# mhozza/covest

Measured on AMD Instinct MI355X. Metric: grid-point log-likelihood evals/s, repeat model, 10k-bin hist, higher is better.
Workload: dtype f64

## Files before the change

### covest_amd/_capi.py

```python
import ctypes
import os
import sys

_HERE = os.path.dirname(os.path.abspath(__file__))
LIB_PATH = os.environ.get("COVEST_AMD_LIB", os.path.join(_HERE, "lib", "libcovest_amd.so"))

MAX_PARAMS = 5
MODEL_BASIC, MODEL_REPEATS = 0, 1
KERNEL_AUTO, KERNEL_DIRECT, KERNEL_RECUR, KERNEL_FACTORED, KERNEL_DIRECT_REF = 0, 1, 2, 3, 4
KERNELS = {"auto": KERNEL_AUTO, "direct": KERNEL_DIRECT, "recur": KERNEL_RECUR,
           "factored": KERNEL_FACTORED, "direct_ref": KERNEL_DIRECT_REF}

EXPORTS = (
    "covest_abi_version", "covest_device_count", "covest_last_error",
    "covest_model_create", "covest_model_destroy", "covest_model_param_count",
    "covest_model_bins_evaluated", "covest_threshold_o", "covest_eval_points", "covest_eval_points_grad", "covest_eval_points_hess",
    "covest_eval_points_opg",
    "covest_probabilities", "covest_reference_overflow", "covest_grid_create", "covest_grid_reset", "covest_grid_destroy", "covest_grid_size",
    "covest_grid_eval", "covest_grid_eval_scan", "covest_grid_scan", "covest_grid_argmin", "covest_grid_axis_min", "covest_grid_argmin_pair_device",
    "covest_grid_ll_device",
    "covest_grid_ll_host",
    "covest_grid_work", "covest_grid_profile", "covest_grid_kernel_ms", "covest_grid_diag",
    "covest_grid_launch_record", "covest_model_launch_record", "covest_compiled_variants",
    "covest_kmer_create", "covest_kmer_destroy", "covest_kmer_reserve", "covest_kmer_add",
    "covest_kmer_add_device", "covest_kmer_histogram", "covest_kmer_slots", "covest_kmer_clear",
    "covest_kmer_count_reads_device", "covest_kmer_partition_info", "covest_kmer_partition_ms", "covest_kmer_memory_limit",
    "covest_kmer_scatter_rate",
    "covest_reads_open", "covest_reads_close", "covest_reads_next", "covest_reads_bytes",
    "covest_thin_histogram", "covest_thin_histogram_timed",
    "covest_truncated_poisson", "covest_truncated_poisson_table",
    "covest_random_genome", "covest_random_genome_device", "covest_simulate_reads", "covest_simulate_reads_device",
    "covest_sample_reads", "covest_sample_reads_device",
    "covest_repeat_plan", "covest_repeat_genome", "covest_repeat_genome_device",
    "covest_draw_thresholds", "covest_draw_histograms", "covest_draw_histograms_device",
    "covest_batch_create", "covest_batch_draw", "covest_batch_counts", "covest_batch_eval_cross", "covest_batch_eval_pairs",
    "covest_batch_argmin_cross", "covest_batch_info", "covest_batch_destroy",
# ... 100 lines not shown
    L.covest_grid_eval.argtypes = [vp, i32, vp]
    L.covest_grid_eval_scan.restype = ctypes.c_int
    L.covest_grid_eval_scan.argtypes = [vp, i32, vp, ctypes.c_double]
    L.covest_grid_scan.restype = ctypes.c_int
    L.covest_grid_scan.argtypes = [vp, i32, ctypes.POINTER(i64), dp, ctypes.POINTER(i32), ctypes.POINTER(i32)]
    L.covest_grid_argmin.restype = ctypes.c_int
    L.covest_grid_argmin.argtypes = [vp, dp, ctypes.POINTER(i64)]
    L.covest_grid_axis_min.restype = ctypes.c_int
    L.covest_grid_axis_min.argtypes = [vp, ctypes.c_uint32, i64, dp, ctypes.POINTER(i64)]
    L.covest_grid_argmin_pair_device.restype = vp
    L.covest_grid_argmin_pair_device.argtypes = [vp]
    L.covest_grid_ll_device.restype = vp
    L.covest_grid_ll_device.argtypes = [vp]
    L.covest_grid_ll_host.restype = ctypes.c_int
    L.covest_grid_ll_host.argtypes = [vp, dp]
    L.covest_grid_work.restype = ctypes.c_int
    L.covest_grid_work.argtypes = [vp, dp, dp, ctypes.POINTER(ctypes.c_char_p)]
    L.covest_grid_profile.restype = ctypes.c_int
    L.covest_grid_profile.argtypes = [vp, i32]
    L.covest_grid_kernel_ms.restype = ctypes.c_int
    L.covest_grid_kernel_ms.argtypes = [vp, dp, ctypes.POINTER(i64)]
    u8p = ctypes.POINTER(ctypes.c_uint8)
    i64p = ctypes.POINTER(i64)
    L.covest_kmer_create.restype = ctypes.c_int
    L.covest_kmer_create.argtypes = [i32, i32, i64, i32, ctypes.POINTER(vp)]
    L.covest_kmer_destroy.restype = None
    L.covest_kmer_destroy.argtypes = [vp]
    L.covest_kmer_reserve.restype = ctypes.c_int
    L.covest_kmer_reserve.argtypes = [vp, i64]
    L.covest_kmer_add.restype = ctypes.c_int
# ... 167 lines not shown
```

### covest_amd/csrc/abi_grid.cpp

```cpp
#include "host.h"

using namespace covest;

namespace covest {

int grid_stage_begin(covest_grid *g, size_t bytes, StageSlot &slot)
{
    if (!g->async_uploads) {
        SharedStage &ss = shared_stage();
        slot.shared_hold = std::unique_lock<std::mutex>(ss.mu);
        HIP_TRY(ss.buf.reserve(bytes));
        slot.ptr = ss.buf.as<char>();
        return COVEST_OK;
    }
    const size_t at = (g->stage_off + 63) / 64 * 64;
    if (at + bytes > g->stage.cap) {
        if (g->stage.ptr)
            g->stage_retired.push_back(std::move(g->stage));
        HIP_TRY(g->stage.reserve(std::max<size_t>(2 * (at + bytes), 1 << 18)));
        slot.ptr = g->stage.as<char>();
        g->stage_off = bytes;
        return COVEST_OK;
    }
    slot.ptr = g->stage.as<char>() + at;
// ... 139 lines not shown

}

static int grid_configure(covest_grid *g, int32_t n_axes, const double *const *axes, const int64_t *axis_len,
                          int64_t flat_begin, int64_t flat_end, const char *who)
{
    covest_model *m = g->model;
    int64_t total = 0, n_values = 0;
    const int arc = check_grid_args(m, n_axes, axes, axis_len, flat_begin, &flat_end, who, &total, &n_values);
    if (arc != COVEST_OK)
        return arc;
    g->configured = false;
    g->flat_begin = flat_begin;
    g->flat_end = flat_end;
    g->evaluated = false;
    g->scan_valid = false;
    g->ev_used = 0;
    g->stage_off = 0;
    const int64_t n = flat_end - flat_begin;
    const int64_t n1 = n_axes == 5 ? axis_len[2] : 1, n2 = n_axes == 5 ? axis_len[3] : 1, n3 = n_axes == 5 ? axis_len[4] : 1;
    const int64_t nq = n_axes == 5 ? n1 * n2 * n3 : 0;

    std::vector<int32_t> table((size_t)nq);
    if (nq)
        threshold_table(m, axes[2], n1, axes[3], n2, axes[4], n3, table.data());

    const GridArena arena(n_values, nq, n);
    char *inputs = nullptr;
    const int src = stage_inputs(g, arena, n_axes, axes, axis_len, table, n, &inputs);
    if (src != COVEST_OK)
// ... 194 lines not shown
    double tsum = 0;
    long long hist[6] = {0, 0, 0, 0, 0, 0};
    for (int64_t i : idx) {
        const long long T = tt[(size_t)((g->src.flat_begin + i) % n_q)];
        tmin = std::min(tmin, T);
        tmax = std::max(tmax, T);
        tsum += (double)T;
        hist[T <= 16 ? 0 : T <= 32 ? 1 : T <= 64 ? 2 : T <= 128 ? 3 : T <= 256 ? 4 : 5]++;
    }
    std::fprintf(stderr, "covest_grid_eval: threshold_o of the queued points: min %lld mean %.1f max %lld; <=16 %lld <=32 %lld <=64 %lld <=128 %lld <=256 %lld more %lld\n",
                 tmin, tsum / queued, tmax, hist[0], hist[1], hist[2], hist[3], hist[4], hist[5]);
    return COVEST_OK;
}
#endif

static int grid_eval(covest_grid *g, int32_t kernel, void *stream, bool scan, double scan_start)
{
    if (!g)
        return fail(COVEST_E_INVALID, "covest_grid_eval: null grid");
    if (!g->configured)
        return fail(COVEST_E_INVALID, "covest_grid_eval: the last covest_grid_reset of this handle failed; reset it again");
    covest_model *m = g->model;
    const int kern = resolve_kernel(m, kernel, g);
    if (kern < 0)
        return kern;
    std::lock_guard<std::mutex> guard(m->lock);
    DeviceGuard dev_guard(m->device);
    int rc = dev_guard.status();
    if (rc != COVEST_OK)
        return rc;
    LaunchRecordScope record(g->record);
    hipStream_t st = static_cast<hipStream_t>(stream);
    const int64_t n = g->flat_end - g->flat_begin;
    if (g->upload_pending && st != nullptr && g->upload_ev)
        HIP_TRY(hipStreamWaitEvent(st, g->upload_ev, 0));
    hipEvent_t bracket_end = nullptr;
    rc = bracket_begin(g, st, &bracket_end);
    if (rc != COVEST_OK)
        return rc;
    HIP_TRY(launch_ll(m, kern, g->src, n, g->ll.as<double>(), sub_list_of(m, g->has_plan ? g->t_max : 2, g->sub_index.ptr, g->sub_word.ptr, g->sub_ctl.ptr), st,
                      &g->last_kernel, g));
    g->last_kernel_id = kern;
    if (bracket_end)
        HIP_TRY(hipEventRecord(bracket_end, st));
#ifdef COVEST_DIAG
    rc = report_queue(g, st, n);
    if (rc != COVEST_OK)
        return rc;
#endif
    if (!g->result_host) {
        static_assert(sizeof(ArgminResult) <= 64 && 64 + sizeof(ScanRecords) <= kPinnedBlockBytes, "pinned block");
        g->result_host = static_cast<ArgminResult *>(pinned_block_take());
        if (!g->result_host)
            return fail(COVEST_E_NOMEM, "covest_grid_eval: no page-locked memory for the result");
    }
    g->scan_valid = scan && n >= 1 && n <= kArgminSmall;
    if (g->scan_valid)
        HIP_TRY(launch_argmin_scan(g->ll.as<double>(), n, g->flat_begin, scan_start, g->result.as<ArgminResult>(), g->result_host,
                                   g->scan_host(), g->sub_ctl.as<unsigned>(), st));
    else
        HIP_TRY(launch_argmin(g->ll.as<double>(), n, g->flat_begin, g->partial_val.as<double>(),
                              g->partial_idx.as<int64_t>(), g->result.as<ArgminResult>(), g->result_host, g->sub_ctl.as<unsigned>(), st));
    g->last_stream = st;
    g->evaluated = true;
    return COVEST_OK;
}

int covest_grid_eval(covest_grid *g, int32_t kernel, void *stream) { return grid_eval(g, kernel, stream, false, 0.0); }

int covest_grid_eval_scan(covest_grid *g, int32_t kernel, void *stream, double start_min)
{
    return grid_eval(g, kernel, stream, true, start_min);
}

int covest_grid_scan(covest_grid *g, int32_t cap, int64_t *index, double *negll, int32_t *n_records, int32_t *truncated)
{
    if (!g || !n_records || !truncated || cap < 0 || (cap > 0 && (!index || !negll)))
        return fail(COVEST_E_INVALID, "covest_grid_scan: bad argument");
    if (!g->evaluated)
        return fail(COVEST_E_INVALID, "covest_grid_scan: covest_grid_eval_scan has not run");
    DeviceGuard dev_guard(g->model->device);
    int rc = dev_guard.status();
    if (rc != COVEST_OK)
        return rc;
    HIP_TRY(hipStreamSynchronize(g->last_stream));
    *n_records = 0;
    *truncated = 1;
// ... 3 lines not shown
    const int32_t have = sr->n;
    *truncated = (sr->truncated || have > cap) ? 1 : 0;
    const int32_t take = std::min(have, cap);
    for (int32_t i = 0; i < take; ++i) {
        index[i] = sr->rec[i].index;
        negll[i] = sr->rec[i].negll;
    }
    *n_records = take;
    return COVEST_OK;
}

int64_t covest_grid_launch_record(const covest_grid *g, char *buf, int64_t cap)
{
    if (!g || cap < 0 || (cap > 0 && !buf))
        return fail(COVEST_E_INVALID, "covest_grid_launch_record: bad argument");
    return launch_record_text(g->record, buf, cap);
}

int covest_grid_argmin(covest_grid *g, double *min_negll, int64_t *argmin_flat)
{
    if (!g || !min_negll || !argmin_flat)
        return fail(COVEST_E_INVALID, "covest_grid_argmin: null argument");
    if (!g->evaluated)
        return fail(COVEST_E_INVALID, "covest_grid_argmin: covest_grid_eval has not run");
    DeviceGuard dev_guard(g->model->device);
    int rc = dev_guard.status();
    if (rc != COVEST_OK)
        return rc;
    HIP_TRY(hipStreamSynchronize(g->last_stream));
    const ArgminResult r = *g->result_host;
    *min_negll = r.min_negll;
    *argmin_flat = r.index < 0 ? -1 : g->flat_begin + r.index;
    return COVEST_OK;
}

int covest_grid_axis_min(covest_grid *g, uint32_t keep_mask, int64_t n_cells, double *min_negll, int64_t *argmin_flat)
{
    if (!g || !min_negll || !argmin_flat)
        return fail(COVEST_E_INVALID, "covest_grid_axis_min: null argument");
    if (!g->evaluated)
        return fail(COVEST_E_INVALID, "covest_grid_axis_min: covest_grid_eval has not run");
    covest_model *m = g->model;
    if (keep_mask >> m->n_par)
        return fail(COVEST_E_INVALID, "covest_grid_axis_min: keep_mask names an axis the grid does not have");
// ... 6 lines not shown
    std::lock_guard<std::mutex> guard(m->lock);
    DeviceGuard dev_guard(m->device);
    int rc = dev_guard.status();
    if (rc != COVEST_OK)
        return rc;
    AxisMinPlan p;
    if (!axis_min_plan(g->len, m->n_par, keep_mask, g->flat_begin, g->flat_end, &p))
        return fail(COVEST_E_INVALID, "covest_grid_axis_min: the axes do not fit a plan");
    const size_t nc = (size_t)n_cells, n_part = p.n_slices > 1 ? nc * (size_t)p.n_slices : 0;
    HIP_TRY(g->axis_buf.reserve(16 * (nc + n_part)));
    double *out_v = g->axis_buf.as<double>();
    int64_t *out_i = reinterpret_cast<int64_t *>(out_v + nc);
    double *part_v = reinterpret_cast<double *>(out_i + nc);
    int64_t *part_i = reinterpret_cast<int64_t *>(part_v + n_part);
    hipStream_t st = g->last_stream;
    HIP_TRY(launch_axis_min(p, g->ll.as<double>(), part_v, part_i, out_v, out_i, st));
    if (16 * nc <= ((size_t)1 << 20)) {
        HIP_TRY(g->axis_host.reserve(16 * nc));
        HIP_TRY(hipMemcpyAsync(g->axis_host.ptr, out_v, 16 * nc, hipMemcpyDeviceToHost, st));
        HIP_TRY(hipStreamSynchronize(st));
        std::memcpy(min_negll, g->axis_host.ptr, 8 * nc);
        std::memcpy(argmin_flat, static_cast<char *>(g->axis_host.ptr) + 8 * nc, 8 * nc);
    } else {
        HIP_TRY(hipStreamSynchronize(st));
        HIP_TRY(hipMemcpy(min_negll, out_v, 8 * nc, hipMemcpyDeviceToHost));
        HIP_TRY(hipMemcpy(argmin_flat, out_i, 8 * nc, hipMemcpyDeviceToHost));
    }
    return COVEST_OK;
}

const double *covest_grid_ll_device(const covest_grid *g) { return g ? g->ll.as<double>() : nullptr; }

const double *covest_grid_argmin_pair_device(const covest_grid *g)
{
    return g ? g->result.as<ArgminResult>()->pair : nullptr;
}

int covest_grid_ll_host(covest_grid *g, double *out_ll)
{
    if (!g || !out_ll)
        return fail(COVEST_E_INVALID, "covest_grid_ll_host: null argument");
    if (!g->evaluated)
        return fail(COVEST_E_INVALID, "covest_grid_ll_host: covest_grid_eval has not run");
    DeviceGuard dev_guard(g->model->device);
    int rc = dev_guard.status();
    if (rc != COVEST_OK)
        return rc;
    const int64_t n = g->flat_end - g->flat_begin;
    HIP_TRY(hipStreamSynchronize(g->last_stream));
    if (n > 0)
        HIP_TRY(hipMemcpy(out_ll, g->ll.ptr, (size_t)n * sizeof(double), hipMemcpyDeviceToHost));
    return COVEST_OK;
}

int64_t covest_grid_diag(covest_grid *g, int64_t *out, int64_t n)
{
    if (!g || !g->has_plan || !g->plan.diag)
        return 0;
// ... 39 lines not shown
```

### covest_amd/csrc/abi_model.cpp

```cpp
#include "host.h"

using namespace covest;

static int check_model_desc(const covest_model_desc *d)
{
    if (d->kind != COVEST_MODEL_BASIC && d->kind != COVEST_MODEL_REPEATS)
        return fail(COVEST_E_INVALID, "covest_model_create: unknown model kind");
    if (d->n_err < 1 || d->n_err > COVEST_MAX_ERROR_CLASSES || d->n_err > d->k + 1)
        return fail(COVEST_E_INVALID, "covest_model_create: n_err must be in 1..min(k+1, 64)");
    if (d->r <= 0 || d->k <= 0)
        return fail(COVEST_E_INVALID, "covest_model_create: k and r must be positive");
    if (d->n_keys < 0 || (d->n_keys > 0 && (!d->keys || !d->counts)) || !d->comb)
        return fail(COVEST_E_INVALID, "covest_model_create: null histogram or comb");
    if (d->kind == COVEST_MODEL_REPEATS && d->n_keys == 0)
        return fail(COVEST_E_INVALID,
                    "covest_model_create: repeats model needs a non-empty histogram "
                    "(max() of an empty dict raises in covest/models.py:186)");
    return COVEST_OK;
}

static void fill_dev_model(DevModel &dm, const covest_model_desc *d, int n_par)
{
    dm.kind = d->kind;
    dm.k = d->k;
// ... 159 lines not shown
        return COVEST_KERNEL_DIRECT_REF;
    case COVEST_KERNEL_RECUR:
        if (basic_fast)
            return COVEST_KERNEL_RECUR;
        return fail(COVEST_E_INVALID, "recurrence kernel needs the basic model, max_error <= 32 and keys in 1..16384");
    case COVEST_KERNEL_FACTORED:
        if (factored_ok || (!g && m->has_tiles && m->dm.kind == COVEST_MODEL_REPEATS && m->dm.n_err <= 8))
            return COVEST_KERNEL_FACTORED;
        return fail(COVEST_E_INVALID, "factored kernel needs the repeats model, keys in 1..16384 and max_error <= 32 "
                                      "(<= 8 for a point list)");
    default:
        return fail(COVEST_E_INVALID, "unknown kernel");
    }
}

static hipError_t launch_factored_grid(covest_grid *g, double *out, const SubList &sub, hipStream_t st)
{
    const covest_model *m = g->model;
    if (g->has_short_part) {
        record_factored_plan(g->plan, g->n_shared_tiles, false);
        hipError_t e = launch_ll_factored(m->dm, m->tv, g->plan, out, sub, st);
        if (e != hipSuccess)
            return e;
        e = launch_ll_fix_list(m->dm, m->tv, g->src, out, sub, st, g->flat_end - g->flat_begin);
        if (e != hipSuccess)
            return e;
    }
    if (g->n_long_tiles > 0) {
        const int64_t n_cols = (int64_t)g->n_long_tiles * 16, n_rows = (int64_t)m->tv.n_items * kTileBins;
        const int64_t ce_begin = g->plan.ce_begin, ce_end = g->plan.ce_end;
        const int64_t per_ce = n_cols * n_rows * (int64_t)sizeof(double);
        const int64_t batch = std::max<int64_t>(1, std::min<int64_t>(ce_end - ce_begin, ((int64_t)1 << 30) / per_ce));
        hipError_t e = g->long_partial.reserve((size_t)(batch * per_ce));
        if (e != hipSuccess)
            return e;
        for (const covest_grid::Part &part : g->long_parts)
            record_factored_plan(part.plan, 0, true);
        for (int64_t first = ce_begin; first < ce_end; first += batch) {
            const int64_t last = std::min(ce_end, first + batch);
// ... 21 lines not shown
{
    SubList l{};
    l.p_clamp = clamp_for(m, t_max);
    l.log_p_clamp = std::log(l.p_clamp);
    l.count = static_cast<unsigned *>(ctl);
    l.index = static_cast<int64_t *>(index);
    l.word = static_cast<unsigned long long *>(word);
    l.index_offset = 0;
#ifdef COVEST_DIAG
    const char *dc = std::getenv("COVEST_DIAG_BASIC_CLASS");
    l.diag_class = dc ? std::atoi(dc) : 0;
#endif
    return l;
}

hipError_t launch_ll(const covest_model *m, int kernel, const PointSource &src, int64_t n, double *out, const SubList &sub,
                     hipStream_t st, const char **name, const covest_grid *g)
{
    if (kernel == COVEST_KERNEL_FACTORED) {
        if (name)
            *name = "ll_factored";
        return launch_factored_grid(const_cast<covest_grid *>(g), out, sub, st);
    }
    if (kernel == COVEST_KERNEL_RECUR) {
        if (name)
            *name = "ll_basic";
        hipError_t e = launch_ll_basic(m->dm, m->tv, src, n, out, sub, st);
        return e != hipSuccess ? e : launch_ll_fix_list(m->dm, m->tv, src, out, sub, st, n);
    }
    if (name)
        *name = kernel == COVEST_KERNEL_DIRECT_REF ? "ll_direct_ref" : "ll_direct";
    return launch_ll_direct(m->dm, src, n, out, nullptr, st, kernel == COVEST_KERNEL_DIRECT_REF);
}

}

constexpr int64_t kInPlaceMaxListPoints = 4;

static int reserve_point_queue(covest_model *m, int64_t n)
{
    HIP_TRY(m->ws_sub_index.reserve((size_t)n * sizeof(int64_t)));
    HIP_TRY(m->ws_sub_word.reserve((size_t)n * sizeof(unsigned long long)));
    HIP_TRY(m->ws_sub_ctl.reserve(sizeof(unsigned)));
    HIP_TRY(hipMemsetAsync(m->ws_sub_ctl.ptr, 0, sizeof(unsigned), nullptr));
    return COVEST_OK;
}

// ... 406 lines not shown
```

### covest_amd/csrc/argmin.hip

```cpp
#include <hip/hip_runtime.h>

#include <algorithm>

#include "cand.h"
#include "kernels.h"
#include "wave.h"

namespace covest {

namespace {

__device__ __forceinline__ Cand block_best(Cand c)
{
    __shared__ double sv[16];
    __shared__ int64_t si[16];
    c = wave_best(c);
    const int lane = threadIdx.x & (kWave - 1), w = threadIdx.x / kWave;
    if (lane == 0) {
        sv[w] = c.v;
        si[w] = c.i;
    }
    __syncthreads();
    const int n_w = blockDim.x / kWave;
    Cand r;
// ... 12 lines not shown
    for (int64_t i = (int64_t)blockIdx.x * blockDim.x + threadIdx.x; i < n; i += stride) {
        const double v = -ll[i];
        if (v < c.v) {
            c.v = v;
            c.i = i;
        }
    }
    c = block_best(c);
    if (threadIdx.x == 0) {
        pv[blockIdx.x] = c.v;
        pi[blockIdx.x] = c.i;
    }
}

__device__ __forceinline__ void publish(Cand c, int64_t flat_begin, ArgminResult *__restrict__ result,
                                        ArgminResult *__restrict__ host_mirror)
{
    ArgminResult r;
    r.min_negll = c.v;
    r.index = (c.i == INT64_MAX) ? -1 : c.i;
    r.pair[0] = c.v;
    r.pair[1] = (c.i == INT64_MAX) ? -1.0 : (double)(flat_begin + c.i);
    *result = r;
    if (host_mirror)
        *host_mirror = r;
}

__global__ __launch_bounds__(256) void argmin_stage2(const double *__restrict__ pv,
                                                     const int64_t *__restrict__ pi, int n_part, int64_t flat_begin,
                                                     ArgminResult *__restrict__ result, ArgminResult *__restrict__ host_mirror,
                                                     unsigned *__restrict__ queue_count)
{
    if (threadIdx.x == 0 && queue_count)
        *queue_count = 0;
    Cand c;
    c.v = INFINITY;
    c.i = INT64_MAX;
    for (int i = threadIdx.x; i < n_part; i += blockDim.x) {
        Cand o;
        o.v = pv[i];
        o.i = pi[i];
        c = better(c, o);
    }
    c = block_best(c);
    if (threadIdx.x == 0)
        publish(c, flat_begin, result, host_mirror);
}

constexpr int kSmallThreads = 1024;

template <class Take>
__device__ __forceinline__ void small_grid_values(const double *__restrict__ ll, int64_t n, Take take)
{
    for (int64_t base = threadIdx.x; base < n; base += 4 * kSmallThreads) {
        double v[4];
#pragma unroll
        for (int u = 0; u < 4; ++u) {
            const int64_t i = base + (int64_t)u * kSmallThreads;
            v[u] = i < n ? -ll[i] : INFINITY;
        }
#pragma unroll
        for (int u = 0; u < 4; ++u) {
            const int64_t i = base + (int64_t)u * kSmallThreads;
            if (i < n)
                take(i, v[u]);
        }
    }
}

__global__ __launch_bounds__(kSmallThreads) void argmin_small(const double *__restrict__ ll, int64_t n, int64_t flat_begin,
                                                             ArgminResult *__restrict__ result, ArgminResult *__restrict__ host_mirror,
                                                             unsigned *__restrict__ queue_count)
{
    if (threadIdx.x == 0 && queue_count)
        *queue_count = 0;
    Cand c;
    c.v = INFINITY;
    c.i = INT64_MAX;
    small_grid_values(ll, n, [&](int64_t i, double v) {
        if (v < c.v) {
            c.v = v;
            c.i = i;
        }
    });
    c = block_best(c);
    if (threadIdx.x == 0)
        publish(c, flat_begin, result, host_mirror);
}

__global__ __launch_bounds__(kSmallThreads) void argmin_scan_small(const double *__restrict__ ll, int64_t n, int64_t flat_begin,
                                                                  double start, ArgminResult *__restrict__ result,
                                                                  ArgminResult *__restrict__ host_mirror,
                                                                  ScanRecords *__restrict__ scan, unsigned *__restrict__ queue_count)
{
    constexpr int NW = kSmallThreads / kWave;
    extern __shared__ double vals[];
    __shared__ double wave_min[NW];
    __shared__ int wave_cnt[NW];
    const int tid = threadIdx.x, lane = tid & (kWave - 1), w = tid / kWave;
    if (tid == 0 && queue_count)
        *queue_count = 0;
    Cand c;
// ... 91 lines not shown
                                           hipFuncAttributeMaxDynamicSharedMemorySize, (int)(kArgminSmall * sizeof(double)));
        if (e != hipSuccess)
            return e;
        raised[dev] = true;
    }
    record_launch(kArgminVariantNames[2]);
    hipLaunchKernelGGL(argmin_scan_small, dim3(1), dim3(kSmallThreads), lds, stream, ll, n, flat_begin, start, result, host_mirror, scan,
                       queue_count);
    return hipGetLastError();
}


hipError_t launch_argmin(const double *ll, int64_t n, int64_t flat_begin, double *partial_val, int64_t *partial_idx,
                         ArgminResult *result, ArgminResult *host_mirror, unsigned *queue_count, hipStream_t stream)
{
    if (n <= kArgminSmall) {
        record_launch(kArgminVariantNames[0]);
        hipLaunchKernelGGL(argmin_small, dim3(1), dim3(kSmallThreads), 0, stream, ll, n, flat_begin, result, host_mirror, queue_count);
        return hipGetLastError();
    }
    const int blocks = (int)std::min<int64_t>(kArgminBlocks, std::max<int64_t>(1, (n + 255) / 256));
    record_launch(kArgminVariantNames[1]);
    hipLaunchKernelGGL(argmin_stage1, dim3(blocks), dim3(256), 0, stream, ll, n, partial_val, partial_idx);
    hipLaunchKernelGGL(argmin_stage2, dim3(1), dim3(256), 0, stream, partial_val, partial_idx, blocks, flat_begin, result,
                       host_mirror, queue_count);
    return hipGetLastError();
}

}
```

### covest_amd/csrc/host.h

```cpp
#pragma once
#include <hip/hip_runtime.h>

#include <algorithm>
#include <cmath>
#include <cstdio>
#include <cstdlib>
#include <cstring>
#include <deque>
#include <limits>
#include <mutex>
#include <new>
#include <optional>
#include <string>
#include <vector>

#include "../../include/covest_amd.h"
#include "device_model.h"
#include "handback.h"
#include "kernels.h"

namespace covest {

int set_error(int code, const std::string &msg);
inline int fail(int code, const std::string &msg) { return set_error(code, msg); }
// ... 227 lines not shown
    int32_t n_shared_tiles = 0;
    std::vector<int32_t> long_q_orig_host;
    DevBuf long_q_orig, long_partial;
    int t_max = 2;
    double q_sum_t_minus_1 = 0.0;
    double contract_flops_per_row = 0.0;
    double sum_t_minus_1 = 0.0;
    LaunchRecord record;
    const char *last_kernel = "none";
    int last_kernel_id = 0;
    hipStream_t last_stream = nullptr;
    ArgminResult *result_host = nullptr;
    ScanRecords *scan_host() const { return reinterpret_cast<ScanRecords *>(reinterpret_cast<char *>(result_host) + 64); }
    bool scan_valid = false;
    bool counter_clean = false;
    HostBuf stage;
    std::vector<HostBuf> stage_retired;
    size_t stage_off = 0;
    bool async_uploads = false;
    bool upload_pending = false;
    hipEvent_t upload_ev = nullptr;
    bool evaluated = false;
    bool configured = false;
    bool profiling = false;
    std::vector<hipEvent_t> ev_begin, ev_end;
    size_t ev_used = 0;
};


struct BulkState {
// ... 62 lines not shown
static_assert(kListLanes + 1 == 513, "include/covest_amd.h documents the largest threshold_o of an uncut point");
double copy_number_weight_host(double q1, double q2, double q, int o);
int build_factored_plan(covest_grid *g, const double *const *axes, const int64_t *axis_len,
                        const std::vector<int32_t> &t_table);
int build_list_plan(covest_model *m, int64_t n, const double *params, const std::vector<int32_t> &t_list,
                    const std::vector<int32_t> *o_base_list, DevBuf &buf, FactoredPlan &pl, bool in_place = false);

int draw_histograms_resident(const char *who, int64_t m, const double *weights, int64_t n_draws, int64_t first_rep,
                             int64_t n_rep, uint64_t seed, DevBuf &d_thr, DevBuf &d_out);

constexpr int64_t kInPlaceMaxPoints = 256;
int resolve_kernel(const covest_model *m, int32_t kernel, const covest_grid *g);
SubList sub_list_of(const covest_model *m, int t_max, void *index, void *word, void *ctl);
hipError_t launch_ll(const covest_model *m, int kernel, const PointSource &src, int64_t n, double *out, const SubList &sub,
                     hipStream_t st, const char **name, const covest_grid *g = nullptr);

}
```

### covest_amd/csrc/host_common.cpp

```cpp
#include "host.h"

using namespace covest;

namespace {
thread_local std::string g_last_error;
}

namespace covest {

int set_error(int code, const std::string &msg)
{
    g_last_error = msg;
    return code;
}

int fail_hip(hipError_t e, const char *what)
{
    g_last_error = std::string(what) + ": " + hipGetErrorString(e);
    if (e == hipErrorOutOfMemory) {
        (void)hipGetLastError();
        return COVEST_E_NOMEM;
    }
    return (e == hipErrorNoDevice || e == hipErrorInvalidDevice || e == hipErrorInsufficientDriver)
               ? COVEST_E_NO_DEVICE
// ... 253 lines not shown
double lgamma_of_factorial(int64_t j)
{
    lgamma_ensure(j);
    return lgamma_at(j);
}

namespace {
thread_local LaunchRecord *tls_record = nullptr;
}

LaunchRecordScope::LaunchRecordScope(LaunchRecord &r) : prev(tls_record)
{
    r.clear();
    tls_record = &r;
}
LaunchRecordScope::~LaunchRecordScope() { tls_record = prev; }

void record_launch(const char *name, int64_t launches)
{
    LaunchRecord *r = tls_record;
    if (!r || launches <= 0)
        return;
    for (int i = 0; i < r->n_entries; ++i)
        if (r->entries[i].name == name) {
            r->entries[i].launches += launches;
            return;
        }
    if (r->n_entries < (int)(sizeof r->entries / sizeof r->entries[0]))
        r->entries[r->n_entries++] = LaunchRecord::Entry{name, launches};
}
// ... 88 lines not shown
```

### covest_amd/csrc/kernels.h

```cpp
#pragma once
#include <hip/hip_runtime_api.h>

#include <cstddef>

#include "device_model.h"
#include "handback.h"
#include "kmer_plan.h"
#include "tiles.h"

namespace covest {

struct LaunchRecord {
    struct Entry {
        const char *name;
        int64_t launches;
    };
    struct Plan {
        int32_t n_threads, n_buf, ld, n_qblocks, shared_tiles, n_pass, list_mode;
        bool long_part;
    };
    Entry entries[16];
    int n_entries = 0;
    Plan plans[8];
    int n_plans = 0;
    void clear() { n_entries = n_plans = 0; }
};
void record_launch(const char *name, int64_t launches = 1);
void record_factored_plan(const FactoredPlan &plan, int shared_tiles, bool long_part);
struct LaunchRecordScope {
    explicit LaunchRecordScope(LaunchRecord &r);
    ~LaunchRecordScope();
    LaunchRecord *prev;
};
constexpr int kFactoredVariants = 10, kBasicVariants = 8, kFixVariants = 6, kArgminVariants = 3, kDerivVariants = 7;
extern const char *const kFactoredVariantNames[kFactoredVariants];
extern const char *const kFactoredFinishNames[2];
extern const char *const kBasicVariantNames[kBasicVariants];
extern const char *const kFixVariantNames[kFixVariants];
extern const char *const kArgminVariantNames[kArgminVariants];
extern const char *const kDerivVariantNames[kDerivVariants];

hipError_t launch_ll_direct(const DevModel &m, const PointSource &src, int64_t n, double *out_ll,
                            double *out_p, hipStream_t stream, bool ref_overflow = false);

hipError_t launch_ll_basic(const DevModel &m, const TileView &tv, const PointSource &src, int64_t n,
// ... 6 lines not shown
                                     const int32_t *first_item, const double *point_par, const int32_t *point_T,
                                     int64_t n_points, double *out_ll, hipStream_t stream);

hipError_t launch_ll_finish_dense(const DevModel &m, const TileView &tv, const PointSource &src, const double *partial,
                                  int64_t ce_first, int64_t n_ce, int64_t n_cols, const int32_t *q_orig, int64_t n_q,
                                  int64_t flat_end, double *out_ll, hipStream_t stream);

hipError_t launch_ll_fix_list(const DevModel &m, const TileView &tv, const PointSource &src, double *ll,
                              const SubList &list, hipStream_t stream, int64_t n_points = 0);

constexpr int kArgminBlocks = 1024;
struct ArgminResult {
    double min_negll;
    int64_t index;
    double pair[2];
};
constexpr int64_t kArgminSmall = 16384;
hipError_t launch_argmin(const double *ll, int64_t n, int64_t flat_begin, double *partial_val, int64_t *partial_idx,
                         ArgminResult *result, ArgminResult *host_mirror, unsigned *queue_count, hipStream_t stream);

constexpr int kScanCap = 120;
struct ScanRecords {
    int32_t n;
    int32_t truncated;
    double start;
    struct {
        int64_t index;
        double negll;
    } rec[kScanCap];
};
hipError_t launch_argmin_scan(const double *ll, int64_t n, int64_t flat_begin, double start, ArgminResult *result,
                              ArgminResult *host_mirror, ScanRecords *scan, unsigned *queue_count, hipStream_t stream);

struct AxisMinPlan {
// ... 171 lines not shown
```

### covest_amd/grid.py

```python
import ctypes
import itertools
import math
import random

import numpy as np

from . import _capi, constants

_DP = ctypes.POINTER(ctypes.c_double)


def partition_flat_range(total, world_size, weights=None, period=None):
    if world_size < 1:
        raise ValueError("world_size must be >= 1")
    if weights is None or total == 0:
        return [(total * r) // world_size for r in range(world_size + 1)]
    w = np.asarray(weights, dtype=np.float64)
    period = len(w) if period is None else period
    assert period == len(w) and total % period == 0
    prefix = np.concatenate(([0.0], np.cumsum(w)))
    per_period = prefix[-1]
    n_periods = total // period
    whole = per_period * n_periods
    bounds = [0]
# ... 97 lines not shown
    return best, arg


class DenseGrid:

    def __init__(self, model, axes, flat_range=None):
        if len(axes) != model.param_count:
            raise ValueError("need one axis per model parameter")
        self.model = model
        ptrs, lens = self._take_axes(axes, flat_range)
        L = _capi.lib()
        h = ctypes.c_void_p()
        _capi.check(L.covest_grid_create(model.handle, len(self.axes), ptrs.ctypes.data, lens.ctypes.data, self.flat_range[0],
                                         self.flat_range[1], ctypes.byref(h)), "covest_grid_create")
        self._handle = h
        if hasattr(model, "_register_grid"):
            model._register_grid(self)

    def _take_axes(self, axes, flat_range):
        parts = [a if type(a) is np.ndarray and a.dtype == np.float64 and a.ndim == 1
                 else np.asarray(a, dtype=np.float64).reshape(-1) for a in axes]
        lens = [p.shape[0] for p in parts]
        flat = np.concatenate(parts) if len(parts) > 1 else np.ascontiguousarray(parts[0])
        self._flat = flat
        self.axes, offs, at = [], [], 0
        for n in lens:
            self.axes.append(flat[at:at + n])
            offs.append(at)
            at += n
        self.shape = tuple(lens)
# ... 58 lines not shown

    def axis_minima(self, keep):
        mask, picked = resolve_keep(self.model.params, keep)
        shape = tuple(self.shape[i] for i in picked)
        val = np.empty(shape, dtype=np.float64)
        idx = np.empty(shape, dtype=np.int64)
        _capi.check(_capi.lib().covest_grid_axis_min(self._handle, mask, val.size, val.ctypes.data_as(_DP),
                                                     idx.ctypes.data_as(ctypes.POINTER(ctypes.c_int64))),
                    "covest_grid_axis_min")
        return val, idx

    def loglikelihoods(self):
        out = np.empty(len(self), dtype=np.float64)
        _capi.check(_capi.lib().covest_grid_ll_host(self._handle, out.ctypes.data_as(_DP)),
                    "covest_grid_ll_host")
        return out

    @property
    def ll_device_ptr(self):
        return _capi.lib().covest_grid_ll_device(self._handle)

    def argmin_pair_tensor(self, device_index):
        import torch
        _capi.require_shared_runtime("DenseGrid.argmin_pair_tensor")
        ptr = _capi.lib().covest_grid_argmin_pair_device(self._handle)

        class _View:
            __cuda_array_interface__ = {"shape": (2,), "typestr": "<f8", "data": (int(ptr), False), "version": 2}

        return torch.as_tensor(_View(), device=torch.device("cuda", device_index))
# ... 247 lines not shown
```

### include/covest_amd.h

```cpp
#ifndef COVEST_AMD_H
#define COVEST_AMD_H

#include <stdint.h>

#ifdef __cplusplus
extern "C" {
#endif

#define COVEST_ABI_VERSION 1

#define COVEST_MODEL_BASIC 0
#define COVEST_MODEL_REPEATS 1
#define COVEST_MAX_PARAMS 5
#define COVEST_MAX_ERROR_CLASSES 64

#define COVEST_OK 0
#define COVEST_E_INVALID (-1)
#define COVEST_E_NO_DEVICE (-2)
#define COVEST_E_HIP (-3)
#define COVEST_E_NOMEM (-4)
#define COVEST_E_UNSUPPORTED (-5)

#define COVEST_KERNEL_AUTO 0
#define COVEST_KERNEL_DIRECT 1
// ... 52 lines not shown
int covest_truncated_poisson(int32_t device, int64_t n, const double *l, const int64_t *j, int32_t mode, double *out);
int covest_truncated_poisson_table(int32_t device, int64_t n_l, const double *l, int64_t n_j, const int64_t *j, double *out);

int covest_probabilities(covest_model *m, const double *params, int32_t clamp, double *out_p);

int covest_grid_create(covest_model *m, int32_t n_axes, const double *const *axes,
                       const int64_t *axis_len, int64_t flat_begin, int64_t flat_end,
                       covest_grid **out);
void covest_grid_destroy(covest_grid *g);
int covest_grid_reset(covest_grid *g, int32_t n_axes, const double *const *axes, const int64_t *axis_len,
                      int64_t flat_begin, int64_t flat_end);
int64_t covest_grid_size(const covest_grid *g);

int covest_grid_eval(covest_grid *g, int32_t kernel, void *stream);

int covest_grid_argmin(covest_grid *g, double *min_negll, int64_t *argmin_flat);

int covest_grid_axis_min(covest_grid *g, uint32_t keep_mask, int64_t n_cells, double *min_negll, int64_t *argmin_flat);

int covest_grid_eval_scan(covest_grid *g, int32_t kernel, void *stream, double start_min);
int covest_grid_scan(covest_grid *g, int32_t cap, int64_t *index, double *negll, int32_t *n_records, int32_t *truncated);

const double *covest_grid_argmin_pair_device(const covest_grid *g);

const double *covest_grid_ll_device(const covest_grid *g);
int covest_grid_ll_host(covest_grid *g, double *out_ll);

int covest_grid_work(const covest_grid *g, double *pmf_terms, double *flops, const char **kernel);

int64_t covest_grid_launch_record(const covest_grid *g, char *buf, int64_t cap);
// ... 90 lines not shown
```

Baseline: 396.1 million.

## Defer the strict fix-list pass until a consumer needs exact log-likelihoods

For recurrence and factored-with-short-part kernels, the grid eval now skips the fix-list relaunch over queued (numerically unsafe) points. Instead, the argmin kernel checks whether any queued point could threaten the provisional winner and flags the result as unproven. The fix pass plus a re-run of argmin then happens lazily, only when the argmin is unproven or the caller reads the log-likelihood arrays, axis mins or the device pair. This adds API surface, a 1024-thread stage2 that scans the queue, and lazy-completion bookkeeping that every accessor must honour.

Result: faster. 413.3 million (median of 6 runs) (+4.4%).

```diff
diff --git a/covest_amd/_capi.py b/covest_amd/_capi.py
--- a/covest_amd/_capi.py
+++ b/covest_amd/_capi.py
@@ -19,7 +19,7 @@
     "covest_probabilities", "covest_reference_overflow", "covest_grid_create", "covest_grid_reset", "covest_grid_destroy", "covest_grid_size",
     "covest_grid_eval", "covest_grid_eval_scan", "covest_grid_scan", "covest_grid_argmin", "covest_grid_axis_min", "covest_grid_argmin_pair_device",
     "covest_grid_ll_device",
-    "covest_grid_ll_host",
+    "covest_grid_ll_host", "covest_grid_complete", "covest_grid_fix_eager", "covest_grid_ll_provisional_host",
     "covest_grid_work", "covest_grid_profile", "covest_grid_kernel_ms", "covest_grid_diag",
     "covest_grid_launch_record", "covest_model_launch_record", "covest_compiled_variants",
     "covest_kmer_create", "covest_kmer_destroy", "covest_kmer_reserve", "covest_kmer_add",
@@ -150,6 +150,12 @@
     L.covest_grid_ll_device.argtypes = [vp]
     L.covest_grid_ll_host.restype = ctypes.c_int
     L.covest_grid_ll_host.argtypes = [vp, dp]
+    L.covest_grid_complete.restype = ctypes.c_int
+    L.covest_grid_complete.argtypes = [vp]
+    L.covest_grid_fix_eager.restype = ctypes.c_int
+    L.covest_grid_fix_eager.argtypes = [vp, ctypes.c_int32]
+    L.covest_grid_ll_provisional_host.restype = ctypes.c_int
+    L.covest_grid_ll_provisional_host.argtypes = [vp, dp]
     L.covest_grid_work.restype = ctypes.c_int
     L.covest_grid_work.argtypes = [vp, dp, dp, ctypes.POINTER(ctypes.c_char_p)]
     L.covest_grid_profile.restype = ctypes.c_int
diff --git a/covest_amd/csrc/abi_grid.cpp b/covest_amd/csrc/abi_grid.cpp
--- a/covest_amd/csrc/abi_grid.cpp
+++ b/covest_amd/csrc/abi_grid.cpp
@@ -177,6 +177,7 @@
     g->flat_begin = flat_begin;
     g->flat_end = flat_end;
     g->evaluated = false;
+    g->fix_pending = false;
     g->scan_valid = false;
     g->ev_used = 0;
     g->stage_off = 0;
@@ -401,6 +402,45 @@
 }
 #endif
 
+static SubList grid_queue(const covest_grid *g, bool put_off)
+{
+    return sub_list_of(g->model, g->has_plan ? g->t_max : 2, g->sub_index.ptr, g->sub_word.ptr,
+                       g->sub_ctl.as<unsigned>() + (put_off ? 1 : 0));
+}
+
+static int grid_complete(covest_grid *g, bool *launched = nullptr)
+{
+    if (launched)
+        *launched = false;
+    if (!g->fix_pending)
+        return COVEST_OK;
+    const covest_model *m = g->model;
+    const int64_t n = g->flat_end - g->flat_begin;
+    hipStream_t st = g->last_stream;
+    LaunchRecordScope record(g->record, true);
+    HIP_TRY(launch_ll_fix_list(m->dm, m->tv, g->src, g->ll.as<double>(), grid_queue(g, true), st, n));
+    HIP_TRY(launch_argmin(g->ll.as<double>(), n, g->flat_begin, g->partial_val.as<double>(), g->partial_idx.as<int64_t>(),
+                          g->result.as<ArgminResult>(), g->result_host, nullptr, st));
+    g->fix_pending = false;
+    if (launched)
+        *launched = true;
+    return COVEST_OK;
+}
+
+static int grid_complete_entry(covest_grid *g, bool *launched = nullptr)
+{
+    if (launched)
+        *launched = false;
+    if (!g->fix_pending)
+        return COVEST_OK;
+    covest_model *m = g->model;
+    std::lock_guard<std::mutex> guard(m->lock);
+    DeviceGuard dev_guard(m->device);
+    if (dev_guard.status() != COVEST_OK)
+        return dev_guard.status();
+    return grid_complete(g, launched);
+}
+
 static int grid_eval(covest_grid *g, int32_t kernel, void *stream, bool scan, double scan_start)
 {
     if (!g)
@@ -421,12 +461,16 @@
     const int64_t n = g->flat_end - g->flat_begin;
     if (g->upload_pending && st != nullptr && g->upload_ev)
         HIP_TRY(hipStreamWaitEvent(st, g->upload_ev, 0));
+    g->fix_pending = false;
+    g->counter_clean = false;
+    const bool hands_back = kern == COVEST_KERNEL_RECUR || (kern == COVEST_KERNEL_FACTORED && g->has_short_part);
+    const bool put_off = hands_back && !scan && !g->fix_eager;
     hipEvent_t bracket_end = nullptr;
     rc = bracket_begin(g, st, &bracket_end);
     if (rc != COVEST_OK)
         return rc;
-    HIP_TRY(launch_ll(m, kern, g->src, n, g->ll.as<double>(), sub_list_of(m, g->has_plan ? g->t_max : 2, g->sub_index.ptr, g->sub_word.ptr, g->sub_ctl.ptr), st,
-                      &g->last_kernel, g));
+    HIP_TRY((put_off ? launch_ll_unfixed : launch_ll)(m, kern, g->src, n, g->ll.as<double>(), grid_queue(g, false), st,
+                                                      &g->last_kernel, g));
     g->last_kernel_id = kern;
     if (bracket_end)
         HIP_TRY(hipEventRecord(bracket_end, st));
@@ -446,8 +490,11 @@
         HIP_TRY(launch_argmin_scan(g->ll.as<double>(), n, g->flat_begin, scan_start, g->result.as<ArgminResult>(), g->result_host,
                                    g->scan_host(), g->sub_ctl.as<unsigned>(), st));
     else
-        HIP_TRY(launch_argmin(g->ll.as<double>(), n, g->flat_begin, g->partial_val.as<double>(),
-                              g->partial_idx.as<int64_t>(), g->result.as<ArgminResult>(), g->result_host, g->sub_ctl.as<unsigned>(), st));
+        HIP_TRY(launch_argmin_proving(g->ll.as<double>(), n, g->flat_begin, g->partial_val.as<double>(),
+                                      g->partial_idx.as<int64_t>(), g->result.as<ArgminResult>(), g->result_host,
+                                      g->sub_ctl.as<unsigned>(), put_off ? g->sub_index.as<int64_t>() : nullptr, st));
+    g->counter_clean = true;
+    g->fix_pending = put_off;
     g->last_stream = st;
     g->evaluated = true;
     return COVEST_OK;
@@ -458,6 +505,22 @@
 int covest_grid_eval_scan(covest_grid *g, int32_t kernel, void *stream, double start_min)
 {
     return grid_eval(g, kernel, stream, true, start_min);
+}
+
+int covest_grid_complete(covest_grid *g)
+{
+    if (!g)
+        return fail(COVEST_E_INVALID, "covest_grid_complete: null grid");
+    return grid_complete_entry(g);
+}
+
+int covest_grid_fix_eager(covest_grid *g, int32_t eager)
+{
+    if (!g)
+        return fail(COVEST_E_INVALID, "covest_grid_fix_eager: null grid");
+    COVEST_TRY(grid_complete_entry(g));
+    g->fix_eager = eager != 0;
+    return COVEST_OK;
 }
 
 int covest_grid_scan(covest_grid *g, int32_t cap, int64_t *index, double *negll, int32_t *n_records, int32_t *truncated)
@@ -491,6 +554,7 @@
 {
     if (!g || cap < 0 || (cap > 0 && !buf))
         return fail(COVEST_E_INVALID, "covest_grid_launch_record: bad argument");
+    COVEST_TRY(grid_complete_entry(const_cast<covest_grid *>(g)));
     return launch_record_text(g->record, buf, cap);
 }
 
@@ -505,6 +569,10 @@
     if (rc != COVEST_OK)
         return rc;
     HIP_TRY(hipStreamSynchronize(g->last_stream));
+    if (g->fix_pending && g->result_host->unproven != 0) {
+        COVEST_TRY(grid_complete_entry(g));
+        HIP_TRY(hipStreamSynchronize(g->last_stream));
+    }
     const ArgminResult r = *g->result_host;
     *min_negll = r.min_negll;
     *argmin_flat = r.index < 0 ? -1 : g->flat_begin + r.index;
@@ -541,6 +609,7 @@
     double *part_v = reinterpret_cast<double *>(out_i + nc);
     int64_t *part_i = reinterpret_cast<int64_t *>(part_v + n_part);
     hipStream_t st = g->last_stream;
+    COVEST_TRY(grid_complete(g));
     HIP_TRY(launch_axis_min(p, g->ll.as<double>(), part_v, part_i, out_v, out_i, st));
     if (16 * nc <= ((size_t)1 << 20)) {
         HIP_TRY(g->axis_host.reserve(16 * nc));
@@ -556,11 +625,30 @@
     return COVEST_OK;
 }
 
-const double *covest_grid_ll_device(const covest_grid *g) { return g ? g->ll.as<double>() : nullptr; }
+const double *covest_grid_ll_device(const covest_grid *g)
+{
+    if (!g)
+        return nullptr;
+    bool launched = false;
+    if (grid_complete_entry(const_cast<covest_grid *>(g), &launched) != COVEST_OK)
+        return nullptr;
+    if (launched) {
+        DeviceGuard dev_guard(g->model->device);
+        if (dev_guard.status() != COVEST_OK || hipStreamSynchronize(g->last_stream) != hipSuccess)
+            return nullptr;
+    }
+    return g->ll.as<double>();
+}
 
 const double *covest_grid_argmin_pair_device(const covest_grid *g)
 {
-    return g ? g->result.as<ArgminResult>()->pair : nullptr;
+    if (!g)
+        return nullptr;
+    covest_grid *gm = const_cast<covest_grid *>(g);
+    if (grid_complete_entry(gm) != COVEST_OK)
+        return nullptr;
+    gm->fix_eager = true;
+    return g->result.as<ArgminResult>()->pair;
 }
 
 int covest_grid_ll_host(covest_grid *g, double *out_ll)
@@ -569,6 +657,24 @@
         return fail(COVEST_E_INVALID, "covest_grid_ll_host: null argument");
     if (!g->evaluated)
         return fail(COVEST_E_INVALID, "covest_grid_ll_host: covest_grid_eval has not run");
+    DeviceGuard dev_guard(g->model->device);
+    int rc = dev_guard.status();
+    if (rc != COVEST_OK)
+        return rc;
+    const int64_t n = g->flat_end - g->flat_begin;
+    COVEST_TRY(grid_complete_entry(g));
+    HIP_TRY(hipStreamSynchronize(g->last_stream));
+    if (n > 0)
+        HIP_TRY(hipMemcpy(out_ll, g->ll.ptr, (size_t)n * sizeof(double), hipMemcpyDeviceToHost));
+    return COVEST_OK;
+}
+
+int covest_grid_ll_provisional_host(covest_grid *g, double *out_ll)
+{
+    if (!g || !out_ll)
+        return fail(COVEST_E_INVALID, "covest_grid_ll_provisional_host: null argument");
+    if (!g->evaluated || !g->fix_pending)
+        return fail(COVEST_E_INVALID, "covest_grid_ll_provisional_host: no strict pass is owed for the last evaluation");
     DeviceGuard dev_guard(g->model->device);
     int rc = dev_guard.status();
     if (rc != COVEST_OK)
diff --git a/covest_amd/csrc/abi_model.cpp b/covest_amd/csrc/abi_model.cpp
--- a/covest_amd/csrc/abi_model.cpp
+++ b/covest_amd/csrc/abi_model.cpp
@@ -197,7 +197,7 @@
     }
 }
 
-static hipError_t launch_factored_grid(covest_grid *g, double *out, const SubList &sub, hipStream_t st)
+static hipError_t launch_factored_grid(covest_grid *g, double *out, const SubList &sub, hipStream_t st, bool with_fix)
 {
     const covest_model *m = g->model;
     if (g->has_short_part) {
@@ -205,7 +205,8 @@
         hipError_t e = launch_ll_factored(m->dm, m->tv, g->plan, out, sub, st);
         if (e != hipSuccess)
             return e;
-        e = launch_ll_fix_list(m->dm, m->tv, g->src, out, sub, st, g->flat_end - g->flat_begin);
+        if (with_fix)
+            e = launch_ll_fix_list(m->dm, m->tv, g->src, out, sub, st, g->flat_end - g->flat_begin);
         if (e != hipSuccess)
             return e;
     }
@@ -257,23 +258,35 @@
     return l;
 }
 
-hipError_t launch_ll(const covest_model *m, int kernel, const PointSource &src, int64_t n, double *out, const SubList &sub,
-                     hipStream_t st, const char **name, const covest_grid *g)
+static hipError_t launch_ll_with(const covest_model *m, int kernel, const PointSource &src, int64_t n, double *out,
+                                 const SubList &sub, hipStream_t st, const char **name, const covest_grid *g, bool with_fix)
 {
     if (kernel == COVEST_KERNEL_FACTORED) {
         if (name)
             *name = "ll_factored";
-        return launch_factored_grid(const_cast<covest_grid *>(g), out, sub, st);
+        return launch_factored_grid(const_cast<covest_grid *>(g), out, sub, st, with_fix);
     }
     if (kernel == COVEST_KERNEL_RECUR) {
         if (name)
             *name = "ll_basic";
         hipError_t e = launch_ll_basic(m->dm, m->tv, src, n, out, sub, st);
-        return e != hipSuccess ? e : launch_ll_fix_list(m->dm, m->tv, src, out, sub, st, n);
+        return e != hipSuccess || !with_fix ? e : launch_ll_fix_list(m->dm, m->tv, src, out, sub, st, n);
     }
     if (name)
         *name = kernel == COVEST_KERNEL_DIRECT_REF ? "ll_direct_ref" : "ll_direct";
     return launch_ll_direct(m->dm, src, n, out, nullptr, st, kernel == COVEST_KERNEL_DIRECT_REF);
+}
+
+hipError_t launch_ll(const covest_model *m, int kernel, const PointSource &src, int64_t n, double *out, const SubList &sub,
+                     hipStream_t st, const char **name, const covest_grid *g)
+{
+    return launch_ll_with(m, kernel, src, n, out, sub, st, name, g, true);
+}
+
+hipError_t launch_ll_unfixed(const covest_model *m, int kernel, const PointSource &src, int64_t n, double *out,
+                             const SubList &sub, hipStream_t st, const char **name, const covest_grid *g)
+{
+    return launch_ll_with(m, kernel, src, n, out, sub, st, name, g, false);
 }
 
 }
diff --git a/covest_amd/csrc/argmin.hip b/covest_amd/csrc/argmin.hip
--- a/covest_amd/csrc/argmin.hip
+++ b/covest_amd/csrc/argmin.hip
@@ -50,11 +50,12 @@
 }
 
 __device__ __forceinline__ void publish(Cand c, int64_t flat_begin, ArgminResult *__restrict__ result,
-                                        ArgminResult *__restrict__ host_mirror)
+                                        ArgminResult *__restrict__ host_mirror, bool unproven = false)
 {
     ArgminResult r;
     r.min_negll = c.v;
     r.index = (c.i == INT64_MAX) ? -1 : c.i;
+    r.unproven = unproven ? 1 : 0;
     r.pair[0] = c.v;
     r.pair[1] = (c.i == INT64_MAX) ? -1.0 : (double)(flat_begin + c.i);
     *result = r;
@@ -62,13 +63,62 @@
         *host_mirror = r;
 }
 
-__global__ __launch_bounds__(256) void argmin_stage2(const double *__restrict__ pv,
+__device__ __forceinline__ void take_queue(unsigned *__restrict__ queue_count, unsigned *s_queued)
+{
+    if (threadIdx.x != 0)
+        return;
+    unsigned q = 0;
+    if (queue_count) {
+        q = queue_count[0];
+        queue_count[1] = q;
+        queue_count[0] = 0;
+    }
+    *s_queued = q;
+}
+
+__device__ __forceinline__ bool winner_unproven(Cand c, const double *__restrict__ ll, const int64_t *__restrict__ queue_index,
+                                                const unsigned *s_queued)
+{
+    __shared__ double win_v;
+    __shared__ int64_t win_i;
+    if (threadIdx.x == 0) {
+        win_v = c.v;
+        win_i = c.i;
+    }
+    __syncthreads();
+    const double v_w = win_v;
+    const int64_t i_w = win_i;
+    const unsigned queued = *s_queued;
+    int threat = 0;
+    if (i_w != INT64_MAX) {
+        const double bound = v_w + 1e-9 * fabs(v_w);
+        for (unsigned base = threadIdx.x; base < queued; base += 4 * blockDim.x) {
+            int64_t i[4];
+            double v[4];
+#pragma unroll
+            for (int u = 0; u < 4; ++u) {
+                const unsigned q = base + (unsigned)u * blockDim.x;
+                i[u] = q < queued ? queue_index[q] : -1;
+            }
+#pragma unroll
+            for (int u = 0; u < 4; ++u)
+                v[u] = i[u] >= 0 ? -ll[i[u]] : INFINITY;
+#pragma unroll
+            for (int u = 0; u < 4; ++u)
+                threat |= (v[u] <= bound || i[u] == i_w) ? 1 : 0;
+        }
+    }
+    return __syncthreads_or(threat) != 0;
+}
+
+__global__ __launch_bounds__(1024) void argmin_stage2(const double *__restrict__ ll, const int64_t *__restrict__ queue_index,
+                                                     const double *__restrict__ pv,
                                                      const int64_t *__restrict__ pi, int n_part, int64_t flat_begin,
                                                      ArgminResult *__restrict__ result, ArgminResult *__restrict__ host_mirror,
                                                      unsigned *__restrict__ queue_count)
 {
-    if (threadIdx.x == 0 && queue_count)
-        *queue_count = 0;
+    __shared__ unsigned s_queued;
+    take_queue(queue_count, &s_queued);
     Cand c;
     c.v = INFINITY;
     c.i = INT64_MAX;
@@ -79,8 +129,9 @@
         c = better(c, o);
     }
     c = block_best(c);
+    const bool unproven = queue_index ? winner_unproven(c, ll, queue_index, &s_queued) : false;
     if (threadIdx.x == 0)
-        publish(c, flat_begin, result, host_mirror);
+        publish(c, flat_begin, result, host_mirror, unproven);
 }
 
 constexpr int kSmallThreads = 1024;
@@ -106,10 +157,10 @@
 
 __global__ __launch_bounds__(kSmallThreads) void argmin_small(const double *__restrict__ ll, int64_t n, int64_t flat_begin,
                                                              ArgminResult *__restrict__ result, ArgminResult *__restrict__ host_mirror,
-                                                             unsigned *__restrict__ queue_count)
-{
-    if (threadIdx.x == 0 && queue_count)
-        *queue_count = 0;
+                                                             unsigned *__restrict__ queue_count, const int64_t *__restrict__ queue_index)
+{
+    __shared__ unsigned s_queued;
+    take_queue(queue_count, &s_queued);
     Cand c;
     c.v = INFINITY;
     c.i = INT64_MAX;
@@ -120,8 +171,9 @@
         }
     });
     c = block_best(c);
+    const bool unproven = queue_index ? winner_unproven(c, ll, queue_index, &s_queued) : false;
     if (threadIdx.x == 0)
-        publish(c, flat_begin, result, host_mirror);
+        publish(c, flat_begin, result, host_mirror, unproven);
 }
 
 __global__ __launch_bounds__(kSmallThreads) void argmin_scan_small(const double *__restrict__ ll, int64_t n, int64_t flat_begin,
@@ -243,16 +295,26 @@
 hipError_t launch_argmin(const double *ll, int64_t n, int64_t flat_begin, double *partial_val, int64_t *partial_idx,
                          ArgminResult *result, ArgminResult *host_mirror, unsigned *queue_count, hipStream_t stream)
 {
+    return launch_argmin_proving(ll, n, flat_begin, partial_val, partial_idx, result, host_mirror, queue_count, nullptr, stream);
+}
+
+hipError_t launch_argmin_proving(const double *ll, int64_t n, int64_t flat_begin, double *partial_val, int64_t *partial_idx,
+                                 ArgminResult *result, ArgminResult *host_mirror, unsigned *queue_count,
+                                 const int64_t *queue_index, hipStream_t stream)
+{
+    if (queue_index && !queue_count)
+        return hipErrorInvalidValue;
     if (n <= kArgminSmall) {
         record_launch(kArgminVariantNames[0]);
-        hipLaunchKernelGGL(argmin_small, dim3(1), dim3(kSmallThreads), 0, stream, ll, n, flat_begin, result, host_mirror, queue_count);
+        hipLaunchKernelGGL(argmin_small, dim3(1), dim3(kSmallThreads), 0, stream, ll, n, flat_begin, result, host_mirror, queue_count,
+                           queue_index);
         return hipGetLastError();
     }
     const int blocks = (int)std::min<int64_t>(kArgminBlocks, std::max<int64_t>(1, (n + 255) / 256));
     record_launch(kArgminVariantNames[1]);
     hipLaunchKernelGGL(argmin_stage1, dim3(blocks), dim3(256), 0, stream, ll, n, partial_val, partial_idx);
-    hipLaunchKernelGGL(argmin_stage2, dim3(1), dim3(256), 0, stream, partial_val, partial_idx, blocks, flat_begin, result,
-                       host_mirror, queue_count);
+    hipLaunchKernelGGL(argmin_stage2, dim3(1), dim3(queue_index ? 1024 : 256), 0, stream, ll, queue_index, partial_val, partial_idx,
+                       blocks, flat_begin, result, host_mirror, queue_count);
     return hipGetLastError();
 }
 
diff --git a/covest_amd/csrc/host.h b/covest_amd/csrc/host.h
--- a/covest_amd/csrc/host.h
+++ b/covest_amd/csrc/host.h
@@ -265,6 +265,7 @@
     ScanRecords *scan_host() const { return reinterpret_cast<ScanRecords *>(reinterpret_cast<char *>(result_host) + 64); }
     bool scan_valid = false;
     bool counter_clean = false;
+    bool fix_pending = false, fix_eager = false;
     HostBuf stage;
     std::vector<HostBuf> stage_retired;
     size_t stage_off = 0;
@@ -357,5 +358,7 @@
 SubList sub_list_of(const covest_model *m, int t_max, void *index, void *word, void *ctl);
 hipError_t launch_ll(const covest_model *m, int kernel, const PointSource &src, int64_t n, double *out, const SubList &sub,
                      hipStream_t st, const char **name, const covest_grid *g = nullptr);
+hipError_t launch_ll_unfixed(const covest_model *m, int kernel, const PointSource &src, int64_t n, double *out,
+                             const SubList &sub, hipStream_t st, const char **name, const covest_grid *g);
 
 }
diff --git a/covest_amd/csrc/host_common.cpp b/covest_amd/csrc/host_common.cpp
--- a/covest_amd/csrc/host_common.cpp
+++ b/covest_amd/csrc/host_common.cpp
@@ -291,6 +291,12 @@
     r.clear();
     tls_record = &r;
 }
+LaunchRecordScope::LaunchRecordScope(LaunchRecord &r, bool append) : prev(tls_record)
+{
+    if (!append)
+        r.clear();
+    tls_record = &r;
+}
 LaunchRecordScope::~LaunchRecordScope() { tls_record = prev; }
 
 void record_launch(const char *name, int64_t launches)
diff --git a/covest_amd/csrc/kernels.h b/covest_amd/csrc/kernels.h
--- a/covest_amd/csrc/kernels.h
+++ b/covest_amd/csrc/kernels.h
@@ -29,6 +29,7 @@
 void record_factored_plan(const FactoredPlan &plan, int shared_tiles, bool long_part);
 struct LaunchRecordScope {
     explicit LaunchRecordScope(LaunchRecord &r);
+    LaunchRecordScope(LaunchRecord &r, bool append);
     ~LaunchRecordScope();
     LaunchRecord *prev;
 };
@@ -65,10 +66,15 @@
     double min_negll;
     int64_t index;
     double pair[2];
+    int64_t unproven;
 };
 constexpr int64_t kArgminSmall = 16384;
 hipError_t launch_argmin(const double *ll, int64_t n, int64_t flat_begin, double *partial_val, int64_t *partial_idx,
                          ArgminResult *result, ArgminResult *host_mirror, unsigned *queue_count, hipStream_t stream);
+
+hipError_t launch_argmin_proving(const double *ll, int64_t n, int64_t flat_begin, double *partial_val, int64_t *partial_idx,
+                                 ArgminResult *result, ArgminResult *host_mirror, unsigned *queue_count,
+                                 const int64_t *queue_index, hipStream_t stream);
 
 constexpr int kScanCap = 120;
 struct ScanRecords {
diff --git a/covest_amd/grid.py b/covest_amd/grid.py
--- a/covest_amd/grid.py
+++ b/covest_amd/grid.py
@@ -1,6 +1,7 @@
 import ctypes
 import itertools
 import math
+import os
 import random
 
 import numpy as np
@@ -135,6 +136,8 @@
         _capi.check(L.covest_grid_create(model.handle, len(self.axes), ptrs.ctypes.data, lens.ctypes.data, self.flat_range[0],
                                          self.flat_range[1], ctypes.byref(h)), "covest_grid_create")
         self._handle = h
+        if os.environ.get("COVEST_GRID_FIX", "") == "eager":
+            self.fix_eager(True)
         if hasattr(model, "_register_grid"):
             model._register_grid(self)
 
@@ -223,6 +226,18 @@
         out = np.empty(len(self), dtype=np.float64)
         _capi.check(_capi.lib().covest_grid_ll_host(self._handle, out.ctypes.data_as(_DP)),
                     "covest_grid_ll_host")
+        return out
+
+    def complete(self):
+        _capi.check(_capi.lib().covest_grid_complete(self._handle), "covest_grid_complete")
+
+    def fix_eager(self, eager=True):
+        _capi.check(_capi.lib().covest_grid_fix_eager(self._handle, 1 if eager else 0), "covest_grid_fix_eager")
+
+    def provisional_loglikelihoods(self):
+        out = np.empty(len(self), dtype=np.float64)
+        _capi.check(_capi.lib().covest_grid_ll_provisional_host(self._handle, out.ctypes.data_as(_DP)),
+                    "covest_grid_ll_provisional_host")
         return out
 
     @property
diff --git a/include/covest_amd.h b/include/covest_amd.h
--- a/include/covest_amd.h
+++ b/include/covest_amd.h
@@ -90,6 +90,10 @@
 
 int covest_grid_eval(covest_grid *g, int32_t kernel, void *stream);
 
+int covest_grid_complete(covest_grid *g);
+int covest_grid_fix_eager(covest_grid *g, int32_t eager);
+int covest_grid_ll_provisional_host(covest_grid *g, double *out_ll);
+
 int covest_grid_argmin(covest_grid *g, double *min_negll, int64_t *argmin_flat);
 
 int covest_grid_axis_min(covest_grid *g, uint32_t keep_mask, int64_t n_cells, double *min_negll, int64_t *argmin_flat);
```
